# ZLkanyo009/Yolo-compression-and-deployment-in-FPGA

Measured on AMD Instinct MI355X. Metric: images/sec slim_yolo_v2 int8 416x416, higher is better.
Workload: dtype int8; 1 GPU; slim_yolo_v2_q_bf int8, batch 64 per GPU, 416x416, 2 classes, conf 0.01; global_batch=64, parallelism=batch-shard x1, streams_per_gpu=4, ring_workgroups_per_launch=128, input=f32, input_batches_rotated=4

## Files before the change

include/yolo355.h:

```cpp
#ifndef YOLO355_H
#define YOLO355_H

#include <stddef.h>
#include <stdint.h>

#ifdef __cplusplus
extern "C" {
#endif

#define Y355_MAX_ANCHORS 16
#define Y355_NUM_LAYERS 10
#define Y355_NUM_TRACKERS 11

#define Y355_OK 0
#define Y355_EINVAL (-1)
#define Y355_EHIP (-2)
#define Y355_ENOTREADY (-3)
#define Y355_ERANGE (-4)
#define Y355_EGUARD (-5)

typedef struct y355_engine y355_engine;

typedef struct y355_config {
    int32_t device_id;
// ... 10 lines not shown
} y355_config;

typedef struct y355_layer_stats {
    int64_t absmax_t;
    int32_t frac_bits;
    int32_t reserved;
    int64_t saturated;
    int64_t guard;
} y355_layer_stats;

const char *y355_last_error(void);
int y355_version(void);

int y355_create(const y355_config *cfg, y355_engine **out);
void y355_destroy(y355_engine *h);
int y355_set_thresholds(y355_engine *h, float conf_thresh, float nms_thresh);
#define Y355_OPT_FUSE_FRONT 1
#define Y355_OPT_RING_WORKGROUPS 2
#define Y355_OPT_FUSE_PAIRS 3
#define Y355_OPT_MAX_CANDIDATES 4
#define Y355_OPT_HEAD_ROUTE 5
#define Y355_HEAD_ROUTE_AUTO 0
#define Y355_HEAD_ROUTE_LARGE 1
int y355_set_option(y355_engine *h, int option, int value);
int y355_max_candidates(y355_engine *h);
int y355_overflow(y355_engine *h, int *overflow);

int y355_load_layer(y355_engine *h, int idx, const int8_t *q_w, const int32_t *q_b,
                    int cout, int cin, int e_w, int e_b);

int y355_set_act_exponents(y355_engine *h, const int32_t *sa);
int y355_get_act_exponents(y355_engine *h, int32_t *sa);
int y355_set_act_exponent(y355_engine *h, int tracker, int32_t exponent);
int y355_set_retune(y355_engine *h, const int32_t *retune);

int y355_input_absmax(y355_engine *h, const float *x_dev, int batch, float *out_max);
int y355_run_layer(y355_engine *h, int idx, int batch, int mode, const float *x_dev);
int y355_set_trackers(y355_engine *h, const float *scale, const int32_t *first_a);
int y355_get_trackers(y355_engine *h, float *scale, int32_t *first_a);
int y355_calibrate(y355_engine *h, const float *x_dev, int batch, int freeze, double momentum, int32_t *sa_out, float *max_out);
int y355_tracker_step(float *scale, int32_t *first_a, float max_abs, int freeze, double momentum, int32_t *exponent);
int y355_layer_stats_get(y355_engine *h, int idx, y355_layer_stats *out);
int y355_get_feature(y355_engine *h, int idx, int batch, int8_t *dst_host);

#define Y355_F_GUARD 1
#define Y355_F_TAP 2
int y355_forward(y355_engine *h, const float *x_dev, int batch, int flags,
                 float *boxes_dev, float *scores_dev, int32_t *cls_dev, int32_t *count_dev);
int y355_set_normalization(y355_engine *h, const float *mean_bgr, const float *std_bgr);
int y355_forward_u8(y355_engine *h, const uint8_t *frames_dev, int batch, int flags,
                    float *boxes_dev, float *scores_dev, int32_t *cls_dev, int32_t *count_dev);
int y355_forward_u8_resized(y355_engine *h, const uint8_t *frames_dev, int src_h, int src_w, int batch, int flags,
                            float *boxes_dev, float *scores_dev, int32_t *cls_dev, int32_t *count_dev,
                            uint8_t *resized_out_dev);
typedef struct y355_frame {
    const uint8_t *data_dev;
    int32_t height, width;
    int64_t row_bytes;
} y355_frame;
int y355_forward_frames(y355_engine *h, const y355_frame *frames , int batch, int flags,
                        float *boxes_dev, float *scores_dev, int32_t *cls_dev, int32_t *count_dev);
int y355_resize_frames(y355_engine *h, const y355_frame *frames, int batch, uint8_t *out_dev );
int y355_forward_host(y355_engine *h, const float *x_host, int batch, int flags,
                      float *boxes, float *scores, int32_t *cls, int32_t *count);
int y355_forward_counters(y355_engine *h, int64_t *saturated, int64_t *guard);
int y355_get_candidates(y355_engine *h, int batch, float *boxes, float *scores, int32_t *cls);
// ... 219 lines not shown
```

yolo-compression-and-deployment-in-fpga_amd/csrc/check_kernels.py:

```python
#!/usr/bin/env python3
import glob
import json
import os
import re
import subprocess
import sys

HERE = os.path.dirname(os.path.abspath(__file__))
SIGFILE = os.path.join(HERE, "ring_signature.json")


def signatures(build):
    out = {}
    for f in sorted(glob.glob(os.path.join(build, "*.s"))):
        name = None
        for line in open(f, errors="replace"):
            m = re.match(r"^(_Z\w+):", line)
            if m:
                name = m.group(1) if any(g in m.group(1) for g in ("conv3x3_i8_ring_kernel", "convpx_kernel", "convr_kernel", "pxpair3r_kernel", "convpxb_kernel")) else None
                if name:
                    out[name] = {"lds_dma": 0, "stores": 0, "mfma": 0, "vmcnt": {}}
                continue
            if not name:
                continue
            if "s_endpgm" in line:
                name = None
                continue
            t = line.strip().split()
            if not t:
                continue
            op = t[0]
            if op.startswith("global_load_lds"):
                out[name]["lds_dma"] += 1
            elif op.startswith("global_store") or op.startswith("buffer_store"):
                out[name]["stores"] += 1
            elif op.startswith("v_mfma"):
                out[name]["mfma"] += 1
            elif op == "s_waitcnt":
                m = re.search(r"vmcnt\((\d+)\)", line)
                if m:
                    out[name]["vmcnt"][m.group(1)] = out[name]["vmcnt"].get(m.group(1), 0) + 1
    return out

GUARDED = ("conv3x3_i8_ring_kernel", "conv1_fast_kernel", "front_kernel", "convpx_kernel", "convr_kernel", "pxpair", "convpxb_kernel")


def main(build):
    bad, seen = [], 0
    for rpt in sorted(glob.glob(os.path.join(build, "*.rpt"))):
        name = None
        for line in open(rpt, errors="replace"):
            m = re.search(r"remark: Function Name: (\S+)", line)
            if m:
                name = m.group(1)
                continue
            m = re.search(r"ScratchSize \[bytes/lane\]: (\d+)", line)
            if m and name:
                if any(g in name for g in GUARDED):
                    seen += 1
                    if int(m.group(1)) != 0:
                        bad.append((os.path.basename(rpt), name, int(m.group(1))))
                name = None
    try:
        ver = subprocess.run(["hipcc", "--version"], capture_output=True, text=True).stdout
        if "7.2" not in ver:
            print("check_kernels: WARNING: validated with ROCm 7.2; this is\n" + ver.strip().splitlines()[0])
    except OSError:
# ... 31 lines not shown
```

yolo-compression-and-deployment-in-fpga_amd/csrc/engine.hip:

```cpp
#include "../../include/yolo355.h"
#include "y355_common.h"
#include "head_nms.h"

#include <algorithm>
#include <cmath>
#include <cstdio>
#include <cstdlib>
#include <cstring>
#include <string>
#include <vector>

static thread_local std::string g_err;
int y355_fail(int code, const std::string &msg) {
    g_err = msg;
    return code;
}
static int fail(int code, const std::string &msg) { return y355_fail(code, msg); }
#define HIPCHK(expr)                                                                      \
    do {                                                                                  \
        hipError_t e_ = (expr);                                                           \
        if (e_ != hipSuccess)                                                             \
            return fail(Y355_EHIP, std::string(#expr) + ": " + hipGetErrorString(e_));    \
    } while (0)

// ... 11 lines not shown
struct LayerDef { int cin, cout, pool, leaky, kid; };
const LayerDef kLayers[10] = {
    {3, 16, 1, 1, -1},
    {16, 32, 1, 1, Y355_K_CONV2},
    {32, 64, 0, 1, Y355_K_CONV3_1},
    {64, 64, 1, 1, Y355_K_CONV3_2},
    {64, 128, 0, 1, Y355_K_CONV4_1},
    {128, 128, 1, 1, Y355_K_CONV4_2},
    {128, 256, 0, 1, Y355_K_CONV5},
    {256, 256, 0, 1, Y355_K_CONV67},
    {256, 256, 0, 1, Y355_K_CONV67},
    {256, 0, 0, 0, Y355_K_PRED},
};
const int kRetuneDefault[10] = {11, 10, 10, 11, 11, 10, 11, 11, 11, 10};

struct Layer {
    int cin = 0, cout = 0, cout_pad = 0, pool = 0, leaky = 0, kid = -1;
    int Hin = 0, Win = 0, Hout = 0, Wout = 0, halo = 1;
    int e_w = 0, e_b = 0;
    bool loaded = false, bias_dirty = true;
    std::vector<int32_t> q_b;
    int8_t *w_dev = nullptr;
    int8_t *wpx_dev = nullptr;
    long long wabs = 0;
    int *bias_dev = nullptr;
    long long *bias_w_dev = nullptr;
    int8_t *out_dev = nullptr;
    size_t out_bytes = 0;
    Requant rq{};
    int frac_bits = 0;
};

int kernels_prepared = 0;
}
int y355_prepare_kernels() {
    if (kernels_prepared) return 0;
    for (int i = 0; i < Y355_K_COUNT; ++i) {
        int e = y355_conv_kernel(i)->prepare();
        if (e) return fail(Y355_EHIP, std::string("hipFuncSetAttribute: ") + hipGetErrorString((hipError_t)e));
    }
    if (int e = y355_prepare_head())
        return fail(Y355_EHIP, std::string("hipFuncSetAttribute(head): ") + hipGetErrorString((hipError_t)e));
    if (int e = y355_prepare_conv_ring())
        return fail(Y355_EHIP, std::string("hipFuncSetAttribute(ring): ") + hipGetErrorString((hipError_t)e));
    if (int e = y355_prepare_pair3())
        return fail(Y355_EHIP, std::string("hipFuncSetAttribute(pair3): ") + hipGetErrorString((hipError_t)e));
    if (int e = y355_prepare_conv_px())
        return fail(Y355_EHIP, std::string("hipFuncSetAttribute(px): ") + hipGetErrorString((hipError_t)e));
    if (int e = y355_prepare_convg())
        return fail(Y355_EHIP, std::string("hipFuncSetAttribute(convg): ") + hipGetErrorString((hipError_t)e));
    kernels_prepared = 1;
    return 0;
}
int y355_cu_count(void) {
    static int cached[64] = {};
    int dev = 0;
    if (hipGetDevice(&dev) != hipSuccess || dev < 0 || dev >= 64) return 256;
    if (!cached[dev]) {
        int n = 0;
        if (hipDeviceGetAttribute(&n, hipDeviceAttributeMultiprocessorCount, dev) != hipSuccess || n <= 0) n = 256;
        cached[dev] = n;
    }
    return cached[dev];
}
namespace {
int prepare_kernels() { return y355_prepare_kernels(); }

int make_requant(int cin_real, int taps, int sa_in, int e_w, int e_b, int sa_out, bool have_out, int act, int retune,
                 const int32_t *q_b, int cout, int cout_pad, Requant *rq, int *frac_bits, std::vector<int32_t> *bias_t,
                 std::vector<long long> *bias_w, long long wabs = 0) {
    const int F = std::max(sa_in + e_w, e_b);
// ... 60 lines not shown
    bool own_stream = false;
    Layer L[10];
    int sa[11];
    bool sa_set[11];
    int retune[10];
    float trk_scale[11] = {};
    int trk_first[11] = {};
    const uint8_t *x_u8 = nullptr;
    FrameStage stage;
    int8_t *w0_dev = nullptr;
    int8_t *wf_dev = nullptr;
    Counters *ctr_dev = nullptr;
    CounterSets ctrs;
    unsigned int *absmax_dev = nullptr;
    int8_t *sink_dev = nullptr;
    unsigned long long *stamps_dev = nullptr;
    int Hs = 0, Ws = 0, N = 0;
    HeadState head;
    float *x_stage = nullptr;
    int stamp_layer = -1;
    int profile = 0;
    int fuse_front = 1;
    int fuse_pairs = 1;
    int l2_batch = 0;
    int l0_batch = 0;
    int ring_wgs = 0;
    hipEvent_t ev[Y355_NUM_TIMERS + 1];
    hipEvent_t kev[Y355_NUM_KERNEL_TIMERS][2];
    bool kev_set[Y355_NUM_KERNEL_TIMERS] = {};
    bool ev_ok = false;
    std::vector<void *> allocs;
};

static int dmalloc(y355_engine *h, void **p, size_t bytes, bool zero) {
    HIPCHK(hipMalloc(p, bytes ? bytes : 16));
    h->allocs.push_back(*p);
    if (zero) HIPCHK(hipMemset(*p, 0, bytes ? bytes : 16));
    return 0;
}
extern "C" void y355_destroy(y355_engine *h) {
    if (!h) return;
    (void)hipSetDevice(h->cfg.device_id);
    if (h->stream) (void)hipStreamSynchronize(h->stream);
    for (void *p : h->allocs) (void)hipFree(p);
    y355_head_destroy(h->head);
    y355_stage_destroy(h->stage);
// ... 81 lines not shown
        if (!ok) rc = fail(Y355_EHIP, "hipEventCreate failed");
    }
    if (rc) {
        std::string keep = g_err;
        y355_destroy(h);
        g_err = keep;
        return rc;
    }
    *out = h;
    return 0;
}

extern "C" int y355_set_option(y355_engine *h, int option, int value) {
    if (!h) return fail(Y355_EINVAL, "null engine");
    switch (option) {
    case Y355_OPT_FUSE_FRONT:
        if (value != 0 && value != 1) return fail(Y355_EINVAL, "Y355_OPT_FUSE_FRONT takes 0 or 1");
        h->fuse_front = value;
        return 0;
    case Y355_OPT_FUSE_PAIRS:
        if (value != 0 && value != 1) return fail(Y355_EINVAL, "Y355_OPT_FUSE_PAIRS takes 0 or 1");
        h->fuse_pairs = value;
        return 0;
    case Y355_OPT_RING_WORKGROUPS:
        if (value < 0 || value > 4096) return fail(Y355_EINVAL, "workgroups per launch out of range");
        h->ring_wgs = value;
        return 0;
    case Y355_OPT_MAX_CANDIDATES:
    case Y355_OPT_HEAD_ROUTE: {
        const bool is_cap = option == Y355_OPT_MAX_CANDIDATES;
        if (int rc = y355_head_check_option(h->N, is_cap, value,
                                            is_cap ? "Y355_OPT_MAX_CANDIDATES: 4096 .. min(anchors per image, 65536)"
                                                   : "Y355_OPT_HEAD_ROUTE takes 0 (auto) or 1 (large)"))
            return rc;
        HIPCHK(hipSetDevice(h->cfg.device_id));
        HIPCHK(hipStreamSynchronize(h->stream));
        if (y355_head_set_option(h->head, is_cap, value)) return fail(Y355_EHIP, "device allocation failed");
        return 0;
    }
    default: return fail(Y355_EINVAL, "unknown option");
    }
}

extern "C" int y355_overflow(y355_engine *h, int *overflow) {
    if (!h || !overflow) return fail(Y355_EINVAL, "null argument");
    HIPCHK(hipSetDevice(h->cfg.device_id));
// ... 41 lines not shown
        if (idx == 1) {
            std::vector<int8_t> ff(16384);
            y355_pack_front(nullptr, q_w, ff.data());
            HIPCHK(hipMemcpy(h->wf_dev + 4096, ff.data() + 4096, 12288, hipMemcpyHostToDevice));
        }
    }
    {
        long long best = 0;
        const size_t per = (size_t)cin * 9;
        for (int c = 0; c < cout; ++c) {
            long long sum = 0;
            for (size_t i = 0; i < per; ++i) sum += std::abs((int)q_w[(size_t)c * per + i]);
            best = std::max(best, sum);
        }
        L.wabs = best;
    }
    if (const size_t pxb = idx > 0 ? y355_px_packed_bytes(L.kid) : 0) {
        std::vector<int8_t> px(pxb);
        if (y355_pack_px(L.kid, q_w, cout, cin, px.data())) {
            if (!L.wpx_dev) {
                if (int rc = dmalloc(h, (void **)&L.wpx_dev, px.size(), false)) return rc;
            }
            HIPCHK(hipMemcpy(L.wpx_dev, px.data(), px.size(), hipMemcpyHostToDevice));
        }
    }
    L.q_b.assign(q_b, q_b + cout);
    L.e_w = e_w;
    L.e_b = e_b;
    L.loaded = true;
    L.bias_dirty = true;
    return 0;
}

extern "C" int y355_set_act_exponents(y355_engine *h, const int32_t *sa) {
    if (!h || !sa) return fail(Y355_EINVAL, "null argument");
    for (int i = 0; i < 11; ++i)
        if (sa[i] < -64 || sa[i] > 64) return fail(Y355_EINVAL, "activation exponent out of range");
    for (int i = 0; i < 11; ++i) {
        if (h->sa_set[i] && h->sa[i] == sa[i]) continue;
        h->sa[i] = sa[i];
        h->sa_set[i] = true;
        if (i < 10) h->L[i].bias_dirty = true;
        if (i > 0) h->L[i - 1].bias_dirty = true;
    }
    return 0;
}
// ... 89 lines not shown
        p.out_halo = L.halo;
        p.tiles_x = (L.Win + ki.tw - 1) / ki.tw;
        p.tiles_y = (L.Hin + ki.th - 1) / ki.th;
        p.nblk = L.cout_pad / ki.bn;
        p.rq = L.rq;
        p.mode = mode;
        p.guard = guard;
#ifdef Y355_EXPERIMENTS
        static const int no_ring_mask = getenv("Y355_NO_RING_MASK") ? atoi(getenv("Y355_NO_RING_MASK")) : 0;
        static const int no_px_mask = getenv("Y355_NO_PX_MASK") ? atoi(getenv("Y355_NO_PX_MASK")) : 0;
#else
        constexpr int no_ring_mask = 0, no_px_mask = 0;
#endif
        if (k == 2 && mode == 0) h->l2_batch = B;
        if (L.wpx_dev && !((no_px_mask >> k) & 1)) {
            ConvParams q = p;
            q.w = L.wpx_dev;
            if (y355_launch_conv_px(L.kid, q, h->stream)) {
                HIPCHK(hipGetLastError());
                h->kev_set[k] = p.ev_start != nullptr;
                return 0;
            }
        }
        if (!((no_ring_mask >> k) & 1) && y355_launch_conv_ring(L.kid, p, h->stream)) {
            HIPCHK(hipGetLastError());
            h->kev_set[k] = p.ev_start != nullptr;
            return 0;
        }
        ki.launch(p, p.tiles_x * p.tiles_y * p.nblk * B, h->stream);
    }
    HIPCHK(hipGetLastError());
    return 0;
}

extern "C" int y355_input_absmax(y355_engine *h, const float *x_dev, int batch, float *out_max) {
    if (!h || !x_dev || !out_max) return fail(Y355_EINVAL, "null argument");
    if (batch < 1 || batch > h->cfg.max_batch) return fail(Y355_EINVAL, "batch out of range");
    HIPCHK(hipSetDevice(h->cfg.device_id));
    HIPCHK(hipMemsetAsync(h->absmax_dev, 0, 16, h->stream));
    y355_launch_absmax(x_dev, (size_t)batch * 3 * h->cfg.height * h->cfg.width, h->absmax_dev, h->stream);
    HIPCHK(hipGetLastError());
    unsigned int bits = 0;
    HIPCHK(hipMemcpyAsync(&bits, h->absmax_dev, 4, hipMemcpyDeviceToHost, h->stream));
    HIPCHK(hipStreamSynchronize(h->stream));
    memcpy(out_max, &bits, 4);
    return 0;
// ... 100 lines not shown
}

extern "C" int y355_get_feature(y355_engine *h, int idx, int batch, int8_t *dst) {
    if (!h || !dst || idx < 0 || idx >= 10) return fail(Y355_EINVAL, "bad argument");
    if (batch < 1 || batch > h->cfg.max_batch) return fail(Y355_EINVAL, "batch out of range");
    HIPCHK(hipSetDevice(h->cfg.device_id));
    if (idx == 0 && batch > h->l0_batch)
        return fail(Y355_ENOTREADY, "conv1's map of the last forward was not written (fused front end): "
                                    "run with y355_set_option(h, Y355_OPT_FUSE_FRONT, 0) to tap it");
    if (idx == 2 && batch > h->l2_batch)
        return fail(Y355_ENOTREADY, "conv3_1's map of the last forward was not written (fused conv3_1 -> conv3_2 + pool): "
                                    "run with y355_set_option(h, Y355_OPT_FUSE_PAIRS, 0) to tap it");
    const Layer &L = h->L[idx];
    const int Hp = L.Hout + 2 * L.halo, Wp = L.Wout + 2 * L.halo, CS = L.cout_pad;
    std::vector<int8_t> tmp((size_t)batch * Hp * Wp * CS);
    HIPCHK(hipStreamSynchronize(h->stream));
    HIPCHK(hipMemcpy(tmp.data(), L.out_dev, tmp.size(), hipMemcpyDeviceToHost));
    for (int b = 0; b < batch; ++b)
        for (int c = 0; c < L.cout; ++c)
            for (int y = 0; y < L.Hout; ++y)
                for (int x = 0; x < L.Wout; ++x)
                    dst[(((size_t)b * L.cout + c) * L.Hout + y) * L.Wout + x] =
                        tmp[(((size_t)b * Hp + y + L.halo) * Wp + x + L.halo) * CS + c];
    return 0;
}

static HeadParams head_params(y355_engine *h, int sa_pred, float *ob, float *os, int *oc, int *on, bool tap) {
    HeadParams p{};
    const Layer &L = h->L[9];
    p.nlev = 1;
    HeadLevel &lv = p.lev[0];
    lv.pred = L.out_dev;
    lv.pred_f = nullptr;
    lv.cstride = L.cout_pad;
    lv.Hs = h->Hs;
    lv.Ws = h->Ws;
    lv.stride = 16.0f;
    lv.dq = std::ldexp(1.0f, -sa_pred);
    for (int i = 0; i < 2 * h->cfg.num_anchors; ++i) lv.anchors[i] = h->cfg.anchors[i];
    p.A = h->cfg.num_anchors;
    p.C = h->cfg.num_classes;
    p.wh_mul = 16.0f;
    p.group_by_area = 0;
    p.Hb = h->Hs;
    p.Wb = h->Ws;
    if (h->N > Y355_NMS_CAP) y355_head_area_bins(p, h->Hs, h->Ws);
// ... 536 lines not shown
```

yolo-compression-and-deployment-in-fpga_amd/csrc/y355_common.h:

```cpp
#pragma once
#include <hip/hip_runtime.h>
#include <stdint.h>
#include <string.h>
#include <functional>
#include <string>
#include <vector>

#include <hip/hip_ext.h>

typedef int v4i __attribute__((ext_vector_type(4)));
typedef float v4f __attribute__((ext_vector_type(4)));
typedef __bf16 v8bf __attribute__((ext_vector_type(8)));
#define Y355_STAMP_ROWS 4096

#define Y355_LAUNCH(kernel, grid, block, lds, stream, e0, e1, ...)                                                       \
    do {                                                                                                                 \
        if ((e0) && (e1)) hipExtLaunchKernelGGL(kernel, grid, block, lds, stream, (hipEvent_t)(e0), (hipEvent_t)(e1), 0, __VA_ARGS__); \
        else hipLaunchKernelGGL(kernel, grid, block, lds, stream, __VA_ARGS__);                                          \
    } while (0)

struct Requant {
    int shl;
    int sh;
    int leaky;
// ... 236 lines not shown
bool y355_launch_conv_px(int kid, const ConvParams &p, hipStream_t s);
int y355_prepare_conv_px(void);
size_t y355_px_packed_bytes(int kid);
bool y355_pack_px(int kid, const int8_t *q_w, int cout, int cin, int8_t *dst);
struct PairParams {
    const int8_t *in;
    int8_t *out;
    const int8_t *w1;
    const int8_t *w2;
    const int *bias1;
    const int *bias2;
    Counters *ctr1, *ctr2;
    Requant rq1, rq2;
    int B, H, W;
    void *ev_start, *ev_stop;
    int grid_limit;
    unsigned long long *stamps;
};
bool y355_pair3_eligible(const Requant &rq1, const Requant &rq2, int H, int W);
bool y355_launch_pair3(const PairParams &p, hipStream_t s);
int y355_prepare_pair3(void);
bool y355_launch_conv_ring(int kid, const ConvParams &p, hipStream_t s);
int y355_prepare_conv_ring(void);

void y355_launch_conv1(const Conv1Params &p, hipStream_t s);
void y355_conv1_tiles(int H, int W, int *tx, int *ty);
void y355_pack_conv1(const int8_t *q_w , int8_t *dst );

struct DevMem {
    std::function<int(void **p, size_t bytes, bool zero)> alloc;
    std::function<void(void *p)> release;
    std::function<int(void *dst, const void *src, size_t bytes, hipStream_t s)> upload;
};
const DevMem &y355_hip_mem(void);

struct HeadLevel {
    const int8_t *pred;
    const float *pred_f;
    int cstride;
    int Hs, Ws;
    float stride;
    float dq;
    float anchors[32];
};
struct HeadParams {
    HeadLevel lev[3];
// ... 198 lines not shown
```

yolo-compression-and-deployment-in-fpga_amd/yolo355/_ffi.py:

```python
import ctypes as C
import os

import torch

_HERE = os.path.dirname(os.path.abspath(__file__))
LIB_PATH = os.path.join(_HERE, "libyolo355.so")
HEADER_PATH = os.path.normpath(os.path.join(_HERE, "..", "..", "include", "yolo355.h"))

MAX_ANCHORS = 16
NUM_TIMERS = 12
NUM_KERNEL_TIMERS = 14
F_GUARD, F_TAP = 1, 2
PIPE_AFTER_STREAM = 0x100
PIPE_DEFAULT_HANDLES = 4
OP_LEAKY, OP_POOL, OP_RELU = 1, 2, 4
OPT_FUSE_FRONT = 1
OPT_RING_WORKGROUPS = 2
OPT_FUSE_PAIRS = 3
NET_OPT_WORKGROUPS = 1
NET_OPT_THIN_RESIDENT = 2
OPT_MAX_CANDIDATES = 4
OPT_HEAD_ROUTE = 5
NET_OPT_MAX_CANDIDATES = 3
NET_OPT_HEAD_ROUTE = 4
HEAD_ROUTE_AUTO = 0
HEAD_ROUTE_LARGE = 1
EINVAL, EHIP, ENOTREADY = -1, -2, -3
ERANGE = -4


class Config(C.Structure):
    _fields_ = [("device_id", C.c_int32), ("height", C.c_int32), ("width", C.c_int32),
                ("num_classes", C.c_int32), ("num_anchors", C.c_int32),
                ("anchors", C.c_float * (2 * MAX_ANCHORS)),
                ("conf_thresh", C.c_float), ("nms_thresh", C.c_float),
                ("max_batch", C.c_int32), ("max_det", C.c_int32), ("stream", C.c_void_p),
                ("own_stream", C.c_int32)]


class NetConfig(C.Structure):
    _fields_ = [("device_id", C.c_int32), ("arch", C.c_int32), ("dtype", C.c_int32),
                ("height", C.c_int32), ("width", C.c_int32),
                ("num_classes", C.c_int32), ("num_anchors", C.c_int32),
                ("anchors", C.c_float * (2 * MAX_ANCHORS)),
                ("conf_thresh", C.c_float), ("nms_thresh", C.c_float),
# ... 30 lines not shown
        super().__init__("yolo355 error %d: %s" % (code, msg))
        self.code = code


_lib = None
P = C.POINTER
_SIGS = {
    "y355_last_error": (C.c_char_p, []),
    "y355_version": (C.c_int, []),
    "y355_create": (C.c_int, [P(Config), P(C.c_void_p)]),
    "y355_destroy": (None, [C.c_void_p]),
    "y355_set_thresholds": (C.c_int, [C.c_void_p, C.c_float, C.c_float]),
    "y355_pack_front_weights": (C.c_int, [C.c_void_p, C.c_void_p, C.c_void_p]),
    "y355_set_option": (C.c_int, [C.c_void_p, C.c_int, C.c_int]),
    "y355_load_layer": (C.c_int, [C.c_void_p, C.c_int, C.c_void_p, C.c_void_p, C.c_int, C.c_int, C.c_int, C.c_int]),
    "y355_set_act_exponents": (C.c_int, [C.c_void_p, P(C.c_int32)]),
    "y355_get_act_exponents": (C.c_int, [C.c_void_p, P(C.c_int32)]),
    "y355_set_act_exponent": (C.c_int, [C.c_void_p, C.c_int, C.c_int32]),
    "y355_set_retune": (C.c_int, [C.c_void_p, P(C.c_int32)]),
    "y355_input_absmax": (C.c_int, [C.c_void_p, C.c_void_p, C.c_int, P(C.c_float)]),
    "y355_run_layer": (C.c_int, [C.c_void_p, C.c_int, C.c_int, C.c_int, C.c_void_p]),
    "y355_layer_stats_get": (C.c_int, [C.c_void_p, C.c_int, P(LayerStats)]),
    "y355_get_feature": (C.c_int, [C.c_void_p, C.c_int, C.c_int, C.c_void_p]),
    "y355_forward": (C.c_int, [C.c_void_p, C.c_void_p, C.c_int, C.c_int, C.c_void_p, C.c_void_p, C.c_void_p, C.c_void_p]),
    "y355_set_normalization": (C.c_int, [C.c_void_p, P(C.c_float), P(C.c_float)]),
    "y355_forward_u8": (C.c_int, [C.c_void_p, C.c_void_p, C.c_int, C.c_int, C.c_void_p, C.c_void_p, C.c_void_p, C.c_void_p]),
    "y355_forward_u8_resized": (C.c_int, [C.c_void_p, C.c_void_p, C.c_int, C.c_int, C.c_int, C.c_int, C.c_void_p, C.c_void_p, C.c_void_p,
                                          C.c_void_p, C.c_void_p]),
    "y355_forward_frames": (C.c_int, [C.c_void_p, P(Frame), C.c_int, C.c_int, C.c_void_p, C.c_void_p, C.c_void_p, C.c_void_p]),
    "y355_resize_frames": (C.c_int, [C.c_void_p, P(Frame), C.c_int, C.c_void_p]),
    "y355_forward_host": (C.c_int, [C.c_void_p, C.c_void_p, C.c_int, C.c_int, C.c_void_p, C.c_void_p, C.c_void_p, C.c_void_p]),
    "y355_forward_counters": (C.c_int, [C.c_void_p, P(C.c_int64), P(C.c_int64)]),
    "y355_get_candidates": (C.c_int, [C.c_void_p, C.c_int, C.c_void_p, C.c_void_p, C.c_void_p]),
    "y355_scale_boxes": (C.c_int, [C.c_void_p, C.c_void_p, C.c_void_p, C.c_void_p, C.c_int]),
    "y355_max_det": (C.c_int, [C.c_void_p]),
    "y355_num_anchors_total": (C.c_int, [C.c_void_p]),
    "y355_conv3x3_i8_fused": (C.c_int, [C.c_int, C.c_void_p, C.c_void_p, C.c_void_p, C.c_int, C.c_int, C.c_int,
                                        C.c_int, C.c_int, C.c_int, C.c_int, C.c_int, C.c_int, C.c_int,
                                        C.c_void_p, P(LayerStats)]),
    "y355_conv3x3_i8_raw": (C.c_int, [C.c_int, C.c_void_p, C.c_void_p, C.c_void_p, C.c_int, C.c_int, C.c_int,
                                      C.c_int, C.c_int, C.c_int, C.c_int, C.c_int, C.c_int, C.c_void_p, P(C.c_int32)]),
    "y355_quantize_input_f32_i8": (C.c_int, [C.c_int, C.c_void_p, C.c_size_t, C.c_int, C.c_void_p, P(C.c_int64)]),
    "y355_maxpool2x2_i8": (C.c_int, [C.c_int, C.c_void_p, C.c_int, C.c_int, C.c_int, C.c_int, C.c_void_p]),
    "y355_reorg_f32": (C.c_int, [C.c_int, C.c_void_p, C.c_int, C.c_int, C.c_int, C.c_int, C.c_int, C.c_void_p]),
    "y355_spp_f32": (C.c_int, [C.c_int, C.c_void_p, C.c_int, C.c_int, C.c_int, C.c_int, C.c_void_p]),
    "y355_conv2d_bf16": (C.c_int, [C.c_int, C.c_void_p, C.c_void_p, C.c_void_p, C.c_void_p, C.c_int, C.c_int, C.c_int,
# ... 157 lines not shown
```

yolo-compression-and-deployment-in-fpga_amd/yolo355/engine.py:

```python
import atexit
import ctypes as C
import weakref

import numpy as np
import torch

from . import _ffi, framelist
from .prep import RETUNE, RangeTracker

NUM_LAYERS = 10
LAYER_NAMES = ["conv1", "conv2", "conv3_1", "conv3_2", "conv4_1", "conv4_2", "conv5", "conv6", "conv7", "pred"]


_live = weakref.WeakSet()


@atexit.register
def _close_all():
    for o in list(_live):
        try:
            o.close()
        except Exception:
            pass

# ... 145 lines not shown
        if x.shape[0] > self.max_batch:
            raise ValueError("batch %d > max_batch %d" % (x.shape[0], self.max_batch))
        return x.to(device=self.device, dtype=torch.float32).contiguous()

    def calibrate(self, x, trackers, freeze=True):
        xd = self._dev_input(x)
        sa, mx = _calibrate_call(self._lib.y355_set_trackers, self._lib.y355_get_trackers, self._lib.y355_calibrate, self._h,
                                 xd, trackers, freeze, self._enter)
        self.calib_max = mx
        return sa

    def layer_stats(self, idx):
        st = _ffi.LayerStats()
        _ffi.check(self._lib.y355_layer_stats_get(self._h, idx, C.byref(st)))
        return dict(absmax_t=st.absmax_t, frac_bits=st.frac_bits, saturated=st.saturated, guard=st.guard)

    def get_feature(self, idx, batch):
        cout = [16, 32, 64, 64, 128, 128, 256, 256, 256, len(self.anchors) * (5 + self.num_classes)][idx]
        div = [2, 4, 4, 8, 8, 16, 16, 16, 16, 16][idx]
        out = np.empty((batch, cout, self.input_size[0] // div, self.input_size[1] // div), dtype=np.int8)
        _ffi.check(self._lib.y355_get_feature(self._h, idx, batch, out.ctypes.data))
        return out

    def _buffers(self, B):
        if self._out is None or self._out[0].shape[0] < B:
            md = self.max_det
            self._out = (torch.empty((self.max_batch, md, 4), dtype=torch.float32, device=self.device),
                         torch.empty((self.max_batch, md), dtype=torch.float32, device=self.device),
                         torch.empty((self.max_batch, md), dtype=torch.int32, device=self.device),
                         torch.zeros((self.max_batch,), dtype=torch.int32, device=self.device))
        return self._out

    def forward_device(self, xd, flags=0, out=None):
        B = xd.shape[0]
        ob, os_, oc, on = out if out is not None else self._buffers(B)
        cur = self._enter()
        _ffi.check(self._lib.y355_forward(self._h, xd.data_ptr(), B, int(flags), ob.data_ptr(), os_.data_ptr(),
                                          oc.data_ptr(), on.data_ptr()))
        self._leave(cur)
        return ob, os_, oc, on

    def forward_frames_device(self, frames, flags=0, out=None):
        if frames.dtype != torch.uint8 or frames.dim() != 4 or frames.shape[3] != 3 or not frames.is_cuda:
            raise ValueError("expected a CUDA uint8 tensor [B,h,w,3]")
        frames = frames.contiguous()
        B = frames.shape[0]
# ... 800 lines not shown
```

Before: 338,400 images/sec.

## Add dedicated persistent MFMA kernel for the prediction-head 3x3 conv

Adds a specialised persistent int8 kernel for the pred layer (256 input channels, up to 48 output channels, 13x13 tiles). It keeps all repacked weights resident in LDS and triple-buffers input slabs through LDS-DMA with counted vmcnt waits, overlapping the next tile's loads with the current tile's MFMAs. Requantisation and staging happen in LDS before coalesced stores. The kernel is enabled by default through a new option and falls back to the generic ring path when the requant parameters do not match. It also adds a raw-feature debug getter and extends the scratch and signature checks to cover the new kernel.

```diff
diff --git a/include/yolo355.h b/include/yolo355.h
--- a/include/yolo355.h
+++ b/include/yolo355.h
@@ -56,6 +56,7 @@
 #define Y355_OPT_HEAD_ROUTE 5
 #define Y355_HEAD_ROUTE_AUTO 0
 #define Y355_HEAD_ROUTE_LARGE 1
+#define Y355_OPT_PRED_KERNEL 6
 int y355_set_option(y355_engine *h, int option, int value);
 int y355_max_candidates(y355_engine *h);
 int y355_overflow(y355_engine *h, int *overflow);
@@ -76,6 +77,7 @@
 int y355_tracker_step(float *scale, int32_t *first_a, float max_abs, int freeze, double momentum, int32_t *exponent);
 int y355_layer_stats_get(y355_engine *h, int idx, y355_layer_stats *out);
 int y355_get_feature(y355_engine *h, int idx, int batch, int8_t *dst_host);
+int y355_get_feature_raw(y355_engine *h, int idx, int batch, int8_t *dst_host, int32_t *dims);
 
 #define Y355_F_GUARD 1
 #define Y355_F_TAP 2
diff --git a/yolo-compression-and-deployment-in-fpga_amd/csrc/check_kernels.py b/yolo-compression-and-deployment-in-fpga_amd/csrc/check_kernels.py
--- a/yolo-compression-and-deployment-in-fpga_amd/csrc/check_kernels.py
+++ b/yolo-compression-and-deployment-in-fpga_amd/csrc/check_kernels.py
@@ -17,7 +17,7 @@
         for line in open(f, errors="replace"):
             m = re.match(r"^(_Z\w+):", line)
             if m:
-                name = m.group(1) if any(g in m.group(1) for g in ("conv3x3_i8_ring_kernel", "convpx_kernel", "convr_kernel", "pxpair3r_kernel", "convpxb_kernel")) else None
+                name = m.group(1) if any(g in m.group(1) for g in ("conv3x3_i8_ring_kernel", "convpx_kernel", "convr_kernel", "pxpair3r_kernel", "convpxb_kernel", "predconv_kernel")) else None
                 if name:
                     out[name] = {"lds_dma": 0, "stores": 0, "mfma": 0, "vmcnt": {}}
                 continue
@@ -42,7 +42,7 @@
                     out[name]["vmcnt"][m.group(1)] = out[name]["vmcnt"].get(m.group(1), 0) + 1
     return out
 
-GUARDED = ("conv3x3_i8_ring_kernel", "conv1_fast_kernel", "front_kernel", "convpx_kernel", "convr_kernel", "pxpair", "convpxb_kernel")
+GUARDED = ("conv3x3_i8_ring_kernel", "conv1_fast_kernel", "front_kernel", "convpx_kernel", "convr_kernel", "pxpair", "convpxb_kernel", "predconv_kernel")
 
 
 def main(build):
diff --git a/yolo-compression-and-deployment-in-fpga_amd/csrc/engine.hip b/yolo-compression-and-deployment-in-fpga_amd/csrc/engine.hip
--- a/yolo-compression-and-deployment-in-fpga_amd/csrc/engine.hip
+++ b/yolo-compression-and-deployment-in-fpga_amd/csrc/engine.hip
@@ -57,6 +57,7 @@
     std::vector<int32_t> q_b;
     int8_t *w_dev = nullptr;
     int8_t *wpx_dev = nullptr;
+    int8_t *wpred_dev = nullptr;
     long long wabs = 0;
     int *bias_dev = nullptr;
     long long *bias_w_dev = nullptr;
@@ -82,6 +83,8 @@
         return fail(Y355_EHIP, std::string("hipFuncSetAttribute(pair3): ") + hipGetErrorString((hipError_t)e));
     if (int e = y355_prepare_conv_px())
         return fail(Y355_EHIP, std::string("hipFuncSetAttribute(px): ") + hipGetErrorString((hipError_t)e));
+    if (int e = y355_prepare_predconv())
+        return fail(Y355_EHIP, std::string("hipFuncSetAttribute(predconv): ") + hipGetErrorString((hipError_t)e));
     if (int e = y355_prepare_convg())
         return fail(Y355_EHIP, std::string("hipFuncSetAttribute(convg): ") + hipGetErrorString((hipError_t)e));
     kernels_prepared = 1;
@@ -188,6 +191,7 @@
     int profile = 0;
     int fuse_front = 1;
     int fuse_pairs = 1;
+    int pred_kernel = 1;
     int l2_batch = 0;
     int l0_batch = 0;
     int ring_wgs = 0;
@@ -315,6 +319,10 @@
         if (value != 0 && value != 1) return fail(Y355_EINVAL, "Y355_OPT_FUSE_PAIRS takes 0 or 1");
         h->fuse_pairs = value;
         return 0;
+    case Y355_OPT_PRED_KERNEL:
+        if (value != 0 && value != 1) return fail(Y355_EINVAL, "Y355_OPT_PRED_KERNEL takes 0 or 1");
+        h->pred_kernel = value;
+        return 0;
     case Y355_OPT_RING_WORKGROUPS:
         if (value < 0 || value > 4096) return fail(Y355_EINVAL, "workgroups per launch out of range");
         h->ring_wgs = value;
@@ -402,6 +410,15 @@
                 if (int rc = dmalloc(h, (void **)&L.wpx_dev, px.size(), false)) return rc;
             }
             HIPCHK(hipMemcpy(L.wpx_dev, px.data(), px.size(), hipMemcpyHostToDevice));
+        }
+    }
+    if (L.kid == Y355_K_PRED) {
+        std::vector<int8_t> pw(y355_pred_packed_bytes());
+        if (y355_pack_pred(q_w, cout, cin, pw.data())) {
+            if (!L.wpred_dev) {
+                if (int rc = dmalloc(h, (void **)&L.wpred_dev, pw.size(), false)) return rc;
+            }
+            HIPCHK(hipMemcpy(L.wpred_dev, pw.data(), pw.size(), hipMemcpyHostToDevice));
         }
     }
     L.q_b.assign(q_b, q_b + cout);
@@ -537,6 +554,15 @@
                 return 0;
             }
         }
+        if (L.wpred_dev && h->pred_kernel) {
+            ConvParams q = p;
+            q.w = L.wpred_dev;
+            if (y355_launch_predconv(q, h->stream)) {
+                HIPCHK(hipGetLastError());
+                h->kev_set[k] = p.ev_start != nullptr;
+                return 0;
+            }
+        }
         if (!((no_ring_mask >> k) & 1) && y355_launch_conv_ring(L.kid, p, h->stream)) {
             HIPCHK(hipGetLastError());
             h->kev_set[k] = p.ev_start != nullptr;
@@ -683,6 +709,18 @@
                 for (int x = 0; x < L.Wout; ++x)
                     dst[(((size_t)b * L.cout + c) * L.Hout + y) * L.Wout + x] =
                         tmp[(((size_t)b * Hp + y + L.halo) * Wp + x + L.halo) * CS + c];
+    return 0;
+}
+
+extern "C" int y355_get_feature_raw(y355_engine *h, int idx, int batch, int8_t *dst, int32_t *dims) {
+    if (!h || idx < 0 || idx >= 10) return fail(Y355_EINVAL, "bad argument");
+    if (batch < 1 || batch > h->cfg.max_batch) return fail(Y355_EINVAL, "batch out of range");
+    const Layer &L = h->L[idx];
+    if (dims) { dims[0] = L.Hout + 2 * L.halo; dims[1] = L.Wout + 2 * L.halo; dims[2] = L.cout_pad; }
+    if (!dst) return 0;
+    HIPCHK(hipSetDevice(h->cfg.device_id));
+    HIPCHK(hipStreamSynchronize(h->stream));
+    HIPCHK(hipMemcpy(dst, L.out_dev, (size_t)batch * (L.Hout + 2 * L.halo) * (L.Wout + 2 * L.halo) * L.cout_pad, hipMemcpyDeviceToHost));
     return 0;
 }
 
diff --git a/yolo-compression-and-deployment-in-fpga_amd/csrc/predconv.hip b/yolo-compression-and-deployment-in-fpga_amd/csrc/predconv.hip
--- /dev/null
+++ b/yolo-compression-and-deployment-in-fpga_amd/csrc/predconv.hip
@@ -0,0 +1,343 @@
+#include "y355_dev.h"
+#include <hip/hip_ext.h>
+#include <type_traits>
+
+using namespace y355dev;
+
+namespace y355pred {
+constexpr int CIN = 256, NCH = CIN / 64, SPC = 9, KS = NCH * SPC;
+constexpr int TH = 13, TW = 13, BM = TH * TW;
+constexpr int NF = 3;
+constexpr int PW = TW + 2, PH = TH + 2, PWL = 16;
+constexpr int SLABB = PH * PWL * 64, NPIECE = PH;
+constexpr int WCH = SPC * NF;
+constexpr int MT_TOT = (BM + 15) / 16;
+constexpr int NSLOT = 3;
+constexpr int OFF_W = NSLOT * SLABB;
+constexpr int OFF_DUMMY = OFF_W + KS * NF * 1024;
+constexpr int OFF_BIAS = OFF_DUMMY + 1024;
+constexpr int SSTR = 80;
+constexpr int OUTC = 64;
+#ifndef PRED_DIAG
+#define PRED_DIAG 0
+#endif
+constexpr int OFF_STAMP = OFF_BIAS + 1024;
+constexpr size_t LDS = OFF_BIAS + 1024 + (PRED_DIAG ? 4096 : 0);
+static_assert(LDS <= 160 * 1024, "LDS of one CU");
+static_assert(MT_TOT * 16 * SSTR <= SLABB, "the output tile is staged in a dead slab slot");
+#ifndef Y355_PRED_NW
+#define Y355_PRED_NW 8
+#endif
+}
+using namespace y355pred;
+
+template <int NW>
+__global__ __launch_bounds__(NW * 64, 1) void predconv_kernel(const ConvParams p, const int total_tiles) {
+    constexpr int NTHR = NW * 64;
+    constexpr int PPW = (NPIECE + NW - 1) / NW;
+    constexpr int WPW = (WCH + NW - 1) / NW;
+    constexpr int MT = (MT_TOT + NW - 1) / NW;
+    constexpr int NITP = (BM * (OUTC / 16) + NTHR - 1) / NTHR;
+    static_assert(NW * (MT - 1) < MT_TOT, "every wave has MT - 1 m-tiles, the first ones MT");
+    extern __shared__ __attribute__((aligned(16))) char smem[];
+    const int tid = threadIdx.x;
+    const int lane = tid & 63;
+    const int wave = __builtin_amdgcn_readfirstlane(tid >> 6);
+    const int li = lane & 15, g = lane >> 4;
+    const int H = p.H, W = p.W;
+    const bool full = wave + NW * (MT - 1) < MT_TOT;
+
+    const int ppx0 = min(lane >> 2, PW - 1);
+    const int pwithin = ((lane & 3) ^ ((lane >> 3) & 3)) << 4;
+    auto decode = [&](int tile, int &b, int &y0, int &x0) {
+        if (p.xcd_share_log2 > 0) {
+            const int gs = 8 << p.xcd_share_log2;
+            if (tile < (total_tiles & ~(gs - 1))) {
+                const int j = tile & (gs - 1);
+                tile = (tile & ~(gs - 1)) | ((j & 7) << p.xcd_share_log2) | (j >> 3);
+            }
+        }
+        x0 = (tile % p.tiles_x) * TW;
+        tile /= p.tiles_x;
+        y0 = (tile % p.tiles_y) * TH;
+        b = tile / p.tiles_y;
+    };
+    auto issue_slab = [&](int b, int y0, int x0, int c, int slot) {
+        const int8_t *inb = p.in + (size_t)b * (H + 2) * (W + 2) * CIN + c * 64;
+#pragma unroll
+        for (int j = 0; j < PPW; ++j) {
+            const int q = wave + NW * j;
+            const int gy = min(y0 + q, H + 1), gx = min(x0 + ppx0, W + 1);
+            const int8_t *src = inb + ((size_t)gy * (W + 2) + gx) * CIN + pwithin;
+            char *dst = (q < NPIECE) ? smem + slot * SLABB + q * 1024 : smem + OFF_DUMMY;
+            glds16(src, dst);
+        }
+    };
+    auto issue_w = [&](int c) {
+#pragma unroll
+        for (int j = 0; j < WPW; ++j) {
+            const int f = wave + NW * j;
+            const bool ok = f < WCH;
+            const int8_t *src = p.w + ((size_t)c * WCH + (ok ? f : 0)) * 1024 + lane * 16;
+            char *dst = ok ? smem + OFF_W + (c * WCH + f) * 1024 : smem + OFF_DUMMY;
+            glds16(src, dst);
+        }
+    };
+
+    int tile = blockIdx.x;
+    if (tile >= total_tiles) return;
+    int nstamp = 0;
+    auto stamp = [&]() {
+#if PRED_DIAG
+        if (lane == 0 && nstamp < 31) ((unsigned long long *)(smem + OFF_STAMP))[wave * 32 + nstamp] = __builtin_amdgcn_s_memrealtime();
+        ++nstamp;
+#endif
+        (void)nstamp;
+    };
+    stamp();
+    int b, y0, x0;
+    decode(tile, b, y0, x0);
+    int s0 = 0;
+    auto slot_of = [&](int c) { const int s = s0 + c; return s >= 2 * NSLOT ? s - 2 * NSLOT : s >= NSLOT ? s - NSLOT : s; };
+    glds16(p.bias_t + min(lane * 4, OUTC - 4), wave == 0 ? smem + OFF_BIAS : smem + OFF_DUMMY);
+    issue_slab(b, y0, x0, 0, 0);
+    issue_w(0);
+    issue_slab(b, y0, x0, 1, 1);
+    issue_w(1);
+    stamp();
+    const Requant rq = p.rq;
+    unsigned int nsat = 0;
+    bool first = true;
+
+    for (;;) {
+        const int ntile = tile + gridDim.x;
+        const bool more = ntile < total_tiles;
+        int b2 = b, y2 = y0, x2 = x0;
+        if (more) decode(ntile, b2, y2, x2);
+        int abase[MT][3];
+        {
+            int li_a = li, g_a = g;
+            asm volatile("" : "+v"(li_a), "+v"(g_a));
+#pragma unroll
+            for (int m = 0; m < MT; ++m) {
+                const int row = min((wave + NW * m) * 16 + li_a, BM - 1);
+                const int oy = row / TW, ox = row % TW;
+#pragma unroll
+                for (int dx = 0; dx < 3; ++dx)
+                    abase[m][dx] = (oy * PWL + ox + dx) * 64 + ((g_a ^ (((ox + dx) >> 1) & 3)) << 4);
+            }
+        }
+        v4i acc[MT][NF];
+        auto chunk = [&](int c, auto mtc) {
+            constexpr int MTC = decltype(mtc)::value;
+            const char *slab = smem + slot_of(c) * SLABB;
+            const char *wb = smem + OFF_W + c * WCH * 1024 + lane * 16;
+            v4i bf[2][NF], af[2][MTC];
+            auto load = [&](int t, int u) {
+                const int ko = (t / 3) * PWL * 64, acol = t % 3;
+#pragma unroll
+                for (int f = 0; f < NF; ++f) bf[u][f] = *(const v4i *)(wb + (t * NF + f) * 1024);
+#pragma unroll
+                for (int m = 0; m < MTC; ++m) af[u][m] = *(const v4i *)(slab + abase[m][acol] + ko);
+            };
+            load(0, 0);
+#pragma unroll
+            for (int t = 0; t < SPC; ++t) {
+                const int cur = t & 1;
+                if (t + 1 < SPC) load(t + 1, cur ^ 1);
+#pragma unroll
+                for (int m = 0; m < MTC; ++m)
+#pragma unroll
+                    for (int f = 0; f < NF; ++f)
+                        acc[m][f] = __builtin_amdgcn_mfma_i32_16x16x64_i8(af[cur][m], bf[cur][f], acc[m][f], 0, 0, 0);
+                if (t + 1 < SPC) {
+                    __builtin_amdgcn_sched_group_barrier(0x008, 1, 0);
+                    __builtin_amdgcn_sched_group_barrier(0x100, NF + MTC, 0);
+                    __builtin_amdgcn_sched_group_barrier(0x008, NF * MTC - 1, 0);
+                }
+            }
+        };
+        auto run_chunk = [&](int c) {
+            if (full) chunk(c, std::integral_constant<int, MT>{});
+            else chunk(c, std::integral_constant<int, MT - 1>{});
+        };
+
+        if (first) wait_vmcnt<PPW + WPW>();
+        else wait_vmcnt<PPW + NITP>();
+        lds_barrier();
+        stamp();
+        if (first) issue_w(2);
+        issue_slab(b, y0, x0, 2, slot_of(2));
+        {
+            const int *bl = (const int *)(smem + OFF_BIAS);
+#pragma unroll
+            for (int f = 0; f < NF; ++f) {
+                const int bv = bl[f * 16 + li];
+#pragma unroll
+                for (int m = 0; m < MT; ++m) acc[m][f] = (v4i){bv, bv, bv, bv};
+            }
+        }
+        run_chunk(0);
+        stamp();
+        if (first) wait_vmcnt<WPW + PPW>();
+        else wait_vmcnt<NITP + PPW>();
+        lds_barrier();
+        stamp();
+        if (first) issue_w(3);
+        issue_slab(b, y0, x0, 3, slot_of(3));
+        run_chunk(1);
+        stamp();
+        if (first) wait_vmcnt<WPW + PPW>();
+        else wait_vmcnt<PPW>();
+        lds_barrier();
+        stamp();
+        if (more) issue_slab(b2, y2, x2, 0, slot_of(4));
+        run_chunk(2);
+        stamp();
+        if (more) wait_vmcnt<PPW>();
+        else wait_vmcnt<0>();
+        lds_barrier();
+        stamp();
+        if (more) issue_slab(b2, y2, x2, 1, slot_of(5));
+        run_chunk(3);
+        stamp();
+        lds_barrier();
+        stamp();
+
+        {
+            int tid_e = threadIdx.x;
+            asm volatile("" : "+v"(tid_e));
+            const int lane_e = tid_e & 63, li_e = lane_e & 15, g_e = lane_e >> 4;
+            const float s_pos = __int_as_float((127 + rq.lk - rq.sh_r) << 23), s_neg = __int_as_float((127 - rq.sh_r) << 23);
+            float spv = s_pos, snv = s_neg, mgv = MAGIC;
+            asm volatile("" : "+v"(spv), "+v"(snv), "+v"(mgv));
+            float ymx = MAGIC, ymn = MAGIC;
+            char *stg = smem + slot_of(3) * SLABB;
+            if (tid_e < MT_TOT * 16) *(v4i *)(stg + tid_e * SSTR + NF * 16) = (v4i){0, 0, 0, 0};
+            auto stage = [&](auto clampc) {
+                constexpr bool CL = decltype(clampc)::value;
+#pragma unroll
+                for (int m = 0; m < MT; ++m) {
+                    if (m == MT - 1 && !full) break;
+#pragma unroll
+                    for (int r = 0; r < 4; ++r) {
+                        const int srow = (wave + NW * m) * 16 + 4 * g_e + r;
+                        float pos[NF], neg[NF];
+#pragma unroll
+                        for (int f = 0; f < NF; ++f) {
+                            int v = acc[m][f][r];
+                            if constexpr (CL) asm volatile("" : "+v"(v));
+                            const float tf = (float)v;
+                            pos[f] = fmaf(tf, spv, mgv);
+                            neg[f] = fmaf(tf, snv, mgv);
+                        }
+                        if constexpr (!CL) {
+                            ymx = vmax3(vmax3(ymx, pos[0], pos[1]), pos[2], pos[2]);
+                            ymn = vmin3(vmin3(ymn, neg[0], neg[1]), neg[2], neg[2]);
+                        }
+#pragma unroll
+                        for (int f = 0; f < NF; ++f) {
+                            unsigned int w;
+                            if constexpr (CL) w = __float_as_uint(__builtin_amdgcn_fmed3f(vmax(pos[f], neg[f]), QLO, QHI));
+                            else max_to_byte<0>(w, pos[f], neg[f]);
+                            *(unsigned char *)(stg + srow * SSTR + f * 16 + li_e) = (unsigned char)w;
+                        }
+                    }
+                }
+            };
+            stage(std::false_type{});
+            const bool clamped = ymx > QHI || ymn < QLO;
+            if (__builtin_amdgcn_ballot_w64(clamped) != 0ull) stage(std::true_type{});
+            stamp();
+            lds_barrier();
+            int8_t *outb = p.out + (size_t)b * H * W * OUTC;
+#pragma unroll
+            for (int j = 0; j < NITP; ++j) {
+                const int it = min(tid_e + j * NTHR, BM * (OUTC / 16) - 1);
+                const int row = it >> 2, cg = it & 3;
+                const int oy = y0 + row / TW, ox = x0 + row % TW;
+                const v4i v = *(const v4i *)(stg + row * SSTR + cg * 16);
+                int8_t *dst = outb + ((size_t)oy * W + ox) * OUTC + cg * 16;
+                if (!(oy < H && ox < W)) dst = p.sink + tid_e * 16;
+                *(v4i *)dst = v;
+            }
+            if (clamped) {
+#pragma unroll
+                for (int m = 0; m < MT; ++m) {
+                    if (m == MT - 1 && !full) break;
+#pragma unroll
+                    for (int r = 0; r < 4; ++r) {
+                        const int srow = (wave + NW * m) * 16 + 4 * g_e + r;
+                        const bool real = srow < BM && y0 + srow / TW < H && x0 + srow % TW < W;
+#pragma unroll
+                        for (int f = 0; f < NF; ++f) {
+                            int v = acc[m][f][r];
+                            asm volatile("" : "+v"(v));
+                            const float tf = (float)v;
+                            const float y = vmax(fmaf(tf, spv, mgv), fmaf(tf, snv, mgv));
+                            nsat += (real && (y > QHI || y < QLO)) ? 1u : 0u;
+                        }
+                    }
+                }
+            }
+        }
+        stamp();
+        first = false;
+        if (!more) break;
+        tile = ntile;
+        b = b2; y0 = y2; x0 = x2;
+        s0 = s0 == NSLOT - 1 ? 0 : s0 + 1;
+    }
+    wait_vmcnt<0>();
+    nstamp = 30;
+    stamp();
+#if PRED_DIAG
+    if (p.stamps && lane < 32 && blockIdx.x < Y355_STAMP_ROWS / NW)
+        p.stamps[(size_t)(blockIdx.x * NW + wave) * 32 + lane] = ((unsigned long long *)(smem + OFF_STAMP))[wave * 32 + lane];
+#endif
+    if (nsat) atomicAdd(&p.ctr->sat, (unsigned long long)nsat);
+}
+
+size_t y355_pred_packed_bytes(void) { return (size_t)KS * NF * 1024; }
+
+bool y355_pack_pred(const int8_t *q_w, int cout, int cin, int8_t *dst) {
+    if (cin != CIN || cout < 1 || cout > NF * 16) return false;
+    for (int ks = 0; ks < KS; ++ks)
+        for (int f = 0; f < NF; ++f) {
+            int8_t *fr = dst + ((size_t)ks * NF + f) * 1024;
+            for (int l = 0; l < 64; ++l) {
+                const int g = l >> 4, n = f * 16 + (l & 15);
+                const int tap = ks % 9, ci0 = 64 * (ks / 9) + 16 * g;
+                for (int kk = 0; kk < 16; ++kk) fr[l * 16 + kk] = n < cout ? q_w[((size_t)n * cin + ci0 + kk) * 9 + tap] : 0;
+            }
+        }
+    return true;
+}
+
+int y355_prepare_predconv(void) {
+    return (int)hipFuncSetAttribute((const void *)predconv_kernel<Y355_PRED_NW>, hipFuncAttributeMaxDynamicSharedMemorySize, (int)LDS);
+}
+
+bool y355_launch_predconv(const ConvParams &p_in, hipStream_t s) {
+    if ((p_in.mode & 0xff) != 0 || p_in.rq.wide || p_in.guard) return false;
+    if (!(p_in.rq.shl == 0 && p_in.rq.sh_l == 0 && p_in.rq.sh_r <= 17 && p_in.rq.neg_mul == 1)) return false;
+    if (p_in.cstride != OUTC || p_in.out_halo != 0 || p_in.H < 1 || p_in.W < 1) return false;
+    ConvParams p = p_in;
+    p.tiles_x = (p.W + TW - 1) / TW;
+    p.tiles_y = (p.H + TH - 1) / TH;
+    p.nblk = 1;
+    const int per_image = p.tiles_x * p.tiles_y;
+    const int total = per_image * p.B;
+    p.xcd_share_log2 = per_image == 8 ? 3 : per_image == 4 ? 2 : per_image == 2 ? 1 : 0;
+    int grid = y355_cu_count();
+    if (p.grid_limit > 0 && p.grid_limit < grid) grid = p.grid_limit;
+    if (grid > total) grid = total;
+    if (p.ev_start && p.ev_stop) {
+        hipEvent_t e0 = (hipEvent_t)p.ev_start, e1 = (hipEvent_t)p.ev_stop;
+        p.ev_start = p.ev_stop = nullptr;
+        hipExtLaunchKernelGGL(predconv_kernel<Y355_PRED_NW>, dim3(grid), dim3(Y355_PRED_NW * 64), LDS, s, e0, e1, 0, p, total);
+    } else {
+        hipLaunchKernelGGL(predconv_kernel<Y355_PRED_NW>, dim3(grid), dim3(Y355_PRED_NW * 64), LDS, s, p, total);
+    }
+    return true;
+}
diff --git a/yolo-compression-and-deployment-in-fpga_amd/csrc/y355_common.h b/yolo-compression-and-deployment-in-fpga_amd/csrc/y355_common.h
--- a/yolo-compression-and-deployment-in-fpga_amd/csrc/y355_common.h
+++ b/yolo-compression-and-deployment-in-fpga_amd/csrc/y355_common.h
@@ -282,6 +282,11 @@
 int y355_prepare_pair3(void);
 bool y355_launch_conv_ring(int kid, const ConvParams &p, hipStream_t s);
 int y355_prepare_conv_ring(void);
+
+bool y355_launch_predconv(const ConvParams &p, hipStream_t s);
+int y355_prepare_predconv(void);
+size_t y355_pred_packed_bytes(void);
+bool y355_pack_pred(const int8_t *q_w, int cout, int cin, int8_t *dst);
 
 void y355_launch_conv1(const Conv1Params &p, hipStream_t s);
 void y355_conv1_tiles(int H, int W, int *tx, int *ty);
diff --git a/yolo-compression-and-deployment-in-fpga_amd/yolo355/_ffi.py b/yolo-compression-and-deployment-in-fpga_amd/yolo355/_ffi.py
--- a/yolo-compression-and-deployment-in-fpga_amd/yolo355/_ffi.py
+++ b/yolo-compression-and-deployment-in-fpga_amd/yolo355/_ffi.py
@@ -21,6 +21,7 @@
 NET_OPT_THIN_RESIDENT = 2
 OPT_MAX_CANDIDATES = 4
 OPT_HEAD_ROUTE = 5
+OPT_PRED_KERNEL = 6
 NET_OPT_MAX_CANDIDATES = 3
 NET_OPT_HEAD_ROUTE = 4
 HEAD_ROUTE_AUTO = 0
@@ -97,6 +98,7 @@
     "y355_run_layer": (C.c_int, [C.c_void_p, C.c_int, C.c_int, C.c_int, C.c_void_p]),
     "y355_layer_stats_get": (C.c_int, [C.c_void_p, C.c_int, P(LayerStats)]),
     "y355_get_feature": (C.c_int, [C.c_void_p, C.c_int, C.c_int, C.c_void_p]),
+    "y355_get_feature_raw": (C.c_int, [C.c_void_p, C.c_int, C.c_int, C.c_void_p, P(C.c_int32)]),
     "y355_forward": (C.c_int, [C.c_void_p, C.c_void_p, C.c_int, C.c_int, C.c_void_p, C.c_void_p, C.c_void_p, C.c_void_p]),
     "y355_set_normalization": (C.c_int, [C.c_void_p, P(C.c_float), P(C.c_float)]),
     "y355_forward_u8": (C.c_int, [C.c_void_p, C.c_void_p, C.c_int, C.c_int, C.c_void_p, C.c_void_p, C.c_void_p, C.c_void_p]),
diff --git a/yolo-compression-and-deployment-in-fpga_amd/yolo355/engine.py b/yolo-compression-and-deployment-in-fpga_amd/yolo355/engine.py
--- a/yolo-compression-and-deployment-in-fpga_amd/yolo355/engine.py
+++ b/yolo-compression-and-deployment-in-fpga_amd/yolo355/engine.py
@@ -191,6 +191,13 @@
         _ffi.check(self._lib.y355_get_feature(self._h, idx, batch, out.ctypes.data))
         return out
 
+    def get_feature_raw(self, idx, batch):
+        dims = (C.c_int32 * 3)()
+        _ffi.check(self._lib.y355_get_feature_raw(self._h, idx, batch, None, dims))
+        out = np.empty((batch, dims[0], dims[1], dims[2]), dtype=np.int8)
+        _ffi.check(self._lib.y355_get_feature_raw(self._h, idx, batch, out.ctypes.data, dims))
+        return out
+
     def _buffers(self, B):
         if self._out is None or self._out[0].shape[0] < B:
             md = self.max_det
```

After: 336,900 images/sec. Within noise of the previous version (-0.4%).
